# songrise/AvatarCraft

Hardware: AMD Instinct MI355X
Metric: rays/sec, 4096-ray batch, 256x256 render (64+64 samples/ray) (higher is better)
Workload: dtype f32

## Files before the change

avatarcraft_amd/csrc/render_worklist.hpp:

```cpp
#pragma once
#include <cstdint>
#include <vector>

#if defined(__HIPCC__) || defined(__CUDACC__)
#define AC_WL_HD __host__ __device__ inline
#else
#define AC_WL_HD inline
#endif

#ifndef AC_XCD_CHUNK
#define AC_XCD_CHUNK 512
#endif
#ifndef AC_WORKLIST_POLICY
#define AC_WORKLIST_POLICY 1
#endif

namespace ac_worklist {

constexpr int XCDS = 8;
constexpr int MAX_ITEMS = 8;
constexpr int HEADER_WORDS = 16;

constexpr uint32_t META_SAMPLING = 1u << 12, META_LAST = 1u << 13;
struct Item { uint32_t ray, meta; };
AC_WL_HD uint32_t make_meta(int c_begin, int c_end, int seq, bool sampling, bool last)
{
    return (uint32_t)c_begin | ((uint32_t)c_end << 4) | ((uint32_t)seq << 8) | (sampling ? META_SAMPLING : 0u) | (last ? META_LAST : 0u);
}
AC_WL_HD int meta_begin(uint32_t m) { return (int)(m & 15u); }
AC_WL_HD int meta_end(uint32_t m) { return (int)((m >> 4) & 15u); }
AC_WL_HD int meta_seq(uint32_t m) { return (int)((m >> 8) & 15u); }

AC_WL_HD int xcd_chunk(int n_rays)
{
    const int xper = ((n_rays + 7) / 8 + 7) & ~7;
    return xper < AC_XCD_CHUNK ? xper : AC_XCD_CHUNK;
}
enum { TICKET_END = -2, TICKET_GAP = -1 };
AC_WL_HD int ticket_to_work(int n_rays, int xchunk, int xcd, int t)
{
    const int k = t / xchunk, base = (k * XCDS + xcd) * xchunk;
    if (base >= n_rays) return TICKET_END;
    const int w = base + (t - k * xchunk);
    return w < n_rays ? w : TICKET_GAP;
}
AC_WL_HD int work_to_ray(int w, int pair_n) { return pair_n ? (w >> 1) + ((w & 1) ? pair_n : 0) : w; }

constexpr int N_POLICIES = 9;
inline const int *policy_split(int policy, bool first_round, int local)
{
    static const int s2222[] = { 2, 2, 2, 2, 0 }, s3221[] = { 3, 2, 2, 1, 0 }, s22211[] = { 2, 2, 2, 1, 1, 0 }, s13211[] = { 1, 3, 2, 1, 1, 0 }, s31211[] = { 3, 1, 2, 1, 1, 0 },
                     s332[] = { 3, 3, 2, 0 }, s4211[] = { 4, 2, 1, 1, 0 }, s3311[] = { 3, 3, 1, 1, 0 }, s431[] = { 4, 3, 1, 0 };
    switch (policy) {
    case 1: return s3221;
    case 2: return s22211;
    case 3: return first_round ? s2222 : s22211;
    case 4: return first_round ? s2222 : ((local & 1) ? s31211 : s13211);
    case 5: return s332;
    case 6: return s4211;
    case 7: return s3311;
    case 8: return s431;
    default: return s2222;
    }
}
inline int split_bounds(const int *split8, int tiles, int b[MAX_ITEMS + 1])
{
    int n = 0, cum = 0;
    b[0] = 0;
    for (int q = 0; split8[q]; ++q) {
        cum += split8[q];
        const int e = (tiles * cum) / 8;
        if (e > b[n]) b[++n] = e;
    }
    return n;
}

inline void build(int n_rays, int tiles, int pair_n, int waves_per_xcd, int policy, std::vector<uint32_t> &out)
{
    out.assign(HEADER_WORDS, 0u);
    if (n_rays <= 0 || tiles < 1) return;
    if (tiles > 15) tiles = 15;
    const int xchunk = xcd_chunk(n_rays);
    std::vector<int> rays;
    uint32_t n_items = 0;
    for (int xcd = 0; xcd < XCDS; ++xcd) {
        rays.clear();
        for (int t = 0;; ++t) {
            const int w = ticket_to_work(n_rays, xchunk, xcd, t);
            if (w == TICKET_END) break;
            if (w != TICKET_GAP) rays.push_back(w);
        }
        out[xcd] = n_items;
        for (int seq = 0; seq < MAX_ITEMS; ++seq)
            for (int local = 0; local < (int)rays.size(); ++local) {
                int b[MAX_ITEMS + 1];
                const int n = split_bounds(policy_split(policy, local < waves_per_xcd, local), tiles, b);
                if (seq >= n) continue;
                out.push_back((uint32_t)work_to_ray(rays[local], pair_n));
                out.push_back(make_meta(b[seq], b[seq + 1], seq, seq == 0, seq + 1 == n));
                ++n_items;
            }
        out[XCDS + xcd] = n_items - out[xcd];
    }
}

}
```

Measured before the change: 5.502 million.

## Add head/tail shape policies for ray worklist splitting and default to s431 tail

Adds a family of shape policies that divide each XCD's rays into a head block and a tail block, each with its own tile-split pattern. The default policy moves from the 3-2-2-1 split to a rule where rays are processed whole when an XCD has no more rays than waves, and otherwise every ray uses a 4-3-1 split. The aim is fewer worklist items and less per-item overhead, such as re-sampling and partial compositing, while keeping some tail splitting for load balance. The risk is worse balance at the end of the batch because the chunks are coarser.

After: 5.531 million, median of 6. About the same (+0.5%).

```diff
diff --git a/avatarcraft_amd/csrc/render_worklist.hpp b/avatarcraft_amd/csrc/render_worklist.hpp
--- a/avatarcraft_amd/csrc/render_worklist.hpp
+++ b/avatarcraft_amd/csrc/render_worklist.hpp
@@ -12,7 +12,7 @@
 #define AC_XCD_CHUNK 512
 #endif
 #ifndef AC_WORKLIST_POLICY
-#define AC_WORKLIST_POLICY 1
+#define AC_WORKLIST_POLICY 16
 #endif
 
 namespace ac_worklist {
@@ -47,6 +47,7 @@
 AC_WL_HD int work_to_ray(int w, int pair_n) { return pair_n ? (w >> 1) + ((w & 1) ? pair_n : 0) : w; }
 
 constexpr int N_POLICIES = 9;
+constexpr int FIRST_SHAPE_POLICY = N_POLICIES, N_SHAPE_POLICIES = 8, N_ALL_POLICIES = N_POLICIES + N_SHAPE_POLICIES;
 inline const int *policy_split(int policy, bool first_round, int local)
 {
     static const int s2222[] = { 2, 2, 2, 2, 0 }, s3221[] = { 3, 2, 2, 1, 0 }, s22211[] = { 2, 2, 2, 1, 1, 0 }, s13211[] = { 1, 3, 2, 1, 1, 0 }, s31211[] = { 3, 1, 2, 1, 1, 0 },
@@ -62,6 +63,30 @@
     case 8: return s431;
     default: return s2222;
     }
+}
+struct ShapeRule { const int *head, *tail; int tail_num, tail_den; };
+inline bool is_shape_policy(int policy) { return policy >= FIRST_SHAPE_POLICY && policy < N_ALL_POLICIES; }
+inline ShapeRule shape_rule(int policy)
+{
+    static const int whole[] = { 8, 0 }, s44[] = { 4, 4, 0 }, s431[] = { 4, 3, 1, 0 }, s3221[] = { 3, 2, 2, 1, 0 }, s4211[] = { 4, 2, 1, 1, 0 }, s521[] = { 5, 2, 1, 0 };
+    switch (policy) {
+    case 10: return { whole, s3221, 1, 1 };
+    case 11: return { whole, s4211, 1, 1 };
+    case 12: return { whole, s521, 1, 1 };
+    case 13: return { s44, s431, 1, 1 };
+    case 14: return { whole, s431, 3, 2 };
+    case 15: return { whole, s431, 2, 1 };
+    case 16: return { whole, s431, 1 << 20, 1 };
+    default: return { whole, s431, 1, 1 };
+    }
+}
+inline int head_rays(const ShapeRule &r, int n_local, int waves_per_xcd, int pair_n)
+{
+    if (n_local <= waves_per_xcd) return n_local;
+    const long tail_rays = ((long)waves_per_xcd * r.tail_num) / r.tail_den;
+    int head = n_local - (int)(tail_rays < n_local ? tail_rays : n_local);
+    if (pair_n) head &= ~1;
+    return head;
 }
 inline int split_bounds(const int *split8, int tiles, int b[MAX_ITEMS + 1])
 {
@@ -91,15 +116,26 @@
             if (w != TICKET_GAP) rays.push_back(w);
         }
         out[xcd] = n_items;
-        for (int seq = 0; seq < MAX_ITEMS; ++seq)
-            for (int local = 0; local < (int)rays.size(); ++local) {
-                int b[MAX_ITEMS + 1];
-                const int n = split_bounds(policy_split(policy, local < waves_per_xcd, local), tiles, b);
-                if (seq >= n) continue;
-                out.push_back((uint32_t)work_to_ray(rays[local], pair_n));
-                out.push_back(make_meta(b[seq], b[seq + 1], seq, seq == 0, seq + 1 == n));
-                ++n_items;
-            }
+        const auto block = [&](int lo, int hi, const int *split8) {
+            int b[MAX_ITEMS + 1];
+            int n = split8 ? split_bounds(split8, tiles, b) : 0;
+            for (int seq = 0; seq < MAX_ITEMS; ++seq)
+                for (int local = lo; local < hi; ++local) {
+                    if (!split8) n = split_bounds(policy_split(policy, local < waves_per_xcd, local), tiles, b);
+                    if (seq >= n) continue;
+                    out.push_back((uint32_t)work_to_ray(rays[local], pair_n));
+                    out.push_back(make_meta(b[seq], b[seq + 1], seq, seq == 0, seq + 1 == n));
+                    ++n_items;
+                }
+        };
+        const int n_local = (int)rays.size();
+        if (is_shape_policy(policy)) {
+            static const int whole[] = { 8, 0 };
+            const ShapeRule rule = shape_rule(policy);
+            const int head = head_rays(rule, n_local, waves_per_xcd, pair_n);
+            block(0, head, n_local <= waves_per_xcd ? whole : rule.head);
+            block(head, n_local, rule.tail);
+        } else block(0, n_local, nullptr);
         out[XCDS + xcd] = n_items - out[xcd];
     }
 }
```
